# grahamstockton87/RayTracingOneWeekendApplication

Hardware: AMD Instinct MI355X
Metric: Msamples/sec (pixels x spp) on RTIOW final scene 1920x1080 (higher is better)
Workload: dtype f64; 1 GPU; book1_final 1920x1080x100spp depth 50 (BASELINE configs[1]); tiles=8x8 px per wave, interleaved over ranks, parallelism=1 GPU, scene_seed=1592598565, render_seed=1, program_ops=1334, reduced=False, variant=0, order=fast (rtk_scene_upload_fast; proven bit-identical), frames_in_flight=1

## Files before the change

raytracingoneweekendapplication_amd/csrc/rtk_optimize.cpp:

```cpp
#include <algorithm>
#include <cmath>
#include <cstdlib>
#include <cstring>
#include <limits>
#include <new>
#include <unordered_set>
#include <utility>
#include <vector>

#include "rtk.h"

namespace {

struct Box {
    double lo[3], hi[3];
    static Box empty() {
        const double inf = std::numeric_limits<double>::infinity();
        return Box{{inf, inf, inf}, {-inf, -inf, -inf}};
    }
    void grow(const Box& o) {
        for (int a = 0; a < 3; a++) {
            lo[a] = std::min(lo[a], o.lo[a]);
            hi[a] = std::max(hi[a], o.hi[a]);
        }
    }
    void grow(double x, double y, double z) {
        const double p[3] = {x, y, z};
        for (int a = 0; a < 3; a++) {
            lo[a] = std::min(lo[a], p[a]);
            hi[a] = std::max(hi[a], p[a]);
        }
    }
    bool valid() const { return lo[0] <= hi[0] && lo[1] <= hi[1] && lo[2] <= hi[2]; }
    double area() const {
        if (!valid()) return 0.0;
        const double dx = hi[0] - lo[0], dy = hi[1] - lo[1], dz = hi[2] - lo[2];
        return 2.0 * (dx * dy + dy * dz + dz * dx);
    }
    double centre(int a) const { return 0.5 * (lo[a] + hi[a]); }
    double distance2(const double p[3]) const {
        double d2 = 0;
        for (int a = 0; a < 3; a++) {
            const double d = p[a] < lo[a] ? lo[a] - p[a] : (p[a] > hi[a] ? p[a] - hi[a] : 0.0);
            d2 += d * d;
        }
        return d2;
    }
};

struct Item {
    int32_t node;
    Box box;
    double cost;
};

struct Holder {
    rtk_scene_desc desc;
    std::vector<rtk_node> nodes;
    std::vector<int32_t> children;
    std::vector<rtk_aabb> boxes;
};

struct Optimizer {
    const rtk_scene_desc& in;
    const rtk_optimize_opts& opts;
    Holder& out;
    std::vector<int32_t> memo;
    std::vector<Box> memo_box;
    std::vector<double> memo_cost;
    std::vector<char> on_stack;
    std::vector<char> memo_media;
    std::vector<int32_t> ref_rank;
    std::vector<char> holds_medium;
    bool keep_media_order = true;
    int32_t n_ordered = 0;
    bool failed = false;
    bool has_media = false;
    double margin = 0.0, tri_margin = 0.0;
    int split_depth = 0;
    bool has_triangles = false;
    int64_t n_bvh_in = 0;

    Optimizer(const rtk_scene_desc& i, const rtk_optimize_opts& o, Holder& h)
        : in(i), opts(o), out(h), memo(size_t(i.n_nodes), -1), memo_box(size_t(i.n_nodes)), memo_cost(size_t(i.n_nodes), 1.0), on_stack(size_t(i.n_nodes), 0), memo_media(size_t(i.n_nodes), 0) {}

    static constexpr double kBoxCost = 1.0;
    static constexpr double kChainCost = 3.0;
    double prim_cost(int32_t kind) const { return opts.prim_cost_scale * base_prim_cost(kind); }
    static double base_prim_cost(int32_t kind) {
        switch (kind) {
            case RTK_NODE_SPHERE: return 2.1;
            case RTK_NODE_QUAD: return 1.75;
            case RTK_NODE_TRIANGLE: return 1.75;
            default: return 4.0;
        }
    }

    int32_t fail_node() {
        failed = true;
        return -1;
    }
    int32_t push_node(int32_t kind, int32_t a, int32_t b, int32_t c) {
        out.nodes.push_back(rtk_node{kind, a, b, c});
        return int32_t(out.nodes.size()) - 1;
    }

    static void pad_axis(double& lo, double& hi) {
        const double delta = 0.0001;
        if (hi - lo < delta) {
            const double padding = delta / 2;
            lo -= padding;
            hi += padding;
        }
    }
    bool primitive_box(const rtk_node& n, Box& b) {
        b = Box::empty();
        if (n.kind == RTK_NODE_SPHERE) {
            if (n.a < 0 || n.a >= in.n_spheres) return false;
            const rtk_sphere& s = in.spheres[n.a];
            const double r = s.radius;
            b.grow(s.center0.x - r, s.center0.y - r, s.center0.z - r);
            b.grow(s.center0.x + r, s.center0.y + r, s.center0.z + r);
            const double ex = s.center0.x + s.center_dir.x, ey = s.center0.y + s.center_dir.y, ez = s.center0.z + s.center_dir.z;
            b.grow(ex - r, ey - r, ez - r);
            b.grow(ex + r, ey + r, ez + r);
        } else if (n.kind == RTK_NODE_QUAD) {
            if (n.a < 0 || n.a >= in.n_quads) return false;
            const rtk_quad& q = in.quads[n.a];
            b.grow(q.Q.x, q.Q.y, q.Q.z);
            b.grow(q.Q.x + q.u.x, q.Q.y + q.u.y, q.Q.z + q.u.z);
            b.grow(q.Q.x + q.v.x, q.Q.y + q.v.y, q.Q.z + q.v.z);
            b.grow(q.Q.x + q.u.x + q.v.x, q.Q.y + q.u.y + q.v.y, q.Q.z + q.u.z + q.v.z);
        } else {
            if (n.a < 0 || n.a >= in.n_triangles) return false;
            const rtk_triangle& t = in.triangles[n.a];
            b.grow(t.p0.x, t.p0.y, t.p0.z);
            b.grow(t.p1.x, t.p1.y, t.p1.z);
            b.grow(t.p2.x, t.p2.y, t.p2.z);
        }
        for (int a = 0; a < 3; a++) pad_axis(b.lo[a], b.hi[a]);
        if (n.kind == RTK_NODE_TRIANGLE) {
            b = grown(b, tri_margin);
        }
        return true;
    }

    bool gather(int32_t node, std::vector<Item>& items, std::unordered_set<int32_t>& present, int depth) {
        if (failed || node < 0 || node >= in.n_nodes || depth > 4096) return !(failed = true);
        const rtk_node& n = in.nodes[node];
        if (n.kind == RTK_NODE_LIST) {
            if (n.a < 0 || n.b < 0 || int64_t(n.a) + n.b > in.n_list_children) return !(failed = true);
            for (int32_t k = 0; k < n.b; k++)
                if (!gather(in.list_children[n.a + k], items, present, depth + 1)) return false;
            return true;
        }
        if (n.kind == RTK_NODE_BVH) {
            n_bvh_in++;
            return gather(n.a, items, present, depth + 1) && gather(n.b, items, present, depth + 1);
        }
        Box b;
        double cost;
        const int32_t o = convert(node, b, cost, depth + 1);
        if (o < 0) return false;
        if (!present.insert(o).second && !memo_media[node]) return true;
        items.push_back(Item{o, b, cost});
        return true;
    }

    int32_t convert(int32_t node, Box& box, double& cost, int depth) {
        if (failed || node < 0 || node >= in.n_nodes || depth > 4096) {
            failed = true;
            return -1;
        }
        if (memo[node] >= 0) {
            box = memo_box[node];
            cost = memo_cost[node];
            if (memo_media[node]) has_media = true;
            return memo[node];
        }
        if (on_stack[node]) {
            failed = true;
            return -1;
        }
        on_stack[node] = 1;
        const rtk_node& n = in.nodes[node];
        int32_t o = -1;
        switch (n.kind) {
            case RTK_NODE_SPHERE:
            case RTK_NODE_QUAD:
            case RTK_NODE_TRIANGLE:
                if (n.kind == RTK_NODE_TRIANGLE) has_triangles = true;
                if (!primitive_box(n, box)) {
                    failed = true;
                    break;
                }
                cost = prim_cost(n.kind);
                o = push_node(n.kind, n.a, n.b, ref_rank[size_t(node)]);
                break;
            case RTK_NODE_LIST:
            case RTK_NODE_BVH: {
                if (keep_media_order && holds_medium[size_t(node)]) {
                    o = ordered_group(node, box, cost, depth);
                    memo_media[node] = 1;
                    has_media = true;
                    break;
                }
                const bool media_before = has_media;
                has_media = false;
                o = build_group(node, box, cost, depth);
                memo_media[node] = has_media ? 1 : 0;
                has_media = has_media || media_before;
                break;
            }
            case RTK_NODE_TRANSLATE: {
                if (n.a < 0 || n.a >= in.n_translates) {
                    failed = true;
                    break;
                }
                Box cb;
                double cc;
                const int32_t child = convert(n.b, cb, cc, depth + 1);
                if (child < 0) break;
                const rtk_vec3& off = in.translates[n.a].offset;
                box = cb;
                box.lo[0] += off.x; box.hi[0] += off.x;
                box.lo[1] += off.y; box.hi[1] += off.y;
                box.lo[2] += off.z; box.hi[2] += off.z;
                cost = cc + kChainCost;
                o = push_node(RTK_NODE_TRANSLATE, n.a, child, 0);
                memo_media[node] = memo_media[n.b];
                break;
            }
            case RTK_NODE_ROTATE_Y: {
                if (n.a < 0 || n.a >= in.n_rotates) {
                    failed = true;
                    break;
                }
                Box cb;
                double cc;
                const int32_t child = convert(n.b, cb, cc, depth + 1);
                if (child < 0) break;
                const double s = in.rotates[n.a].sin_theta, c = in.rotates[n.a].cos_theta;
                box = Box::empty();
                for (int i = 0; i < 2; i++)
                    for (int j = 0; j < 2; j++)
                        for (int k = 0; k < 2; k++) {
                            const double x = i ? cb.hi[0] : cb.lo[0], y = j ? cb.hi[1] : cb.lo[1], z = k ? cb.hi[2] : cb.lo[2];
                            box.grow(c * x + s * z, y, -s * x + c * z);
                        }
                cost = cc + kChainCost;
                o = push_node(RTK_NODE_ROTATE_Y, n.a, child, 0);
                memo_media[node] = memo_media[n.b];
                break;
            }
            case RTK_NODE_MEDIUM: {
                if (n.a < 0 || n.a >= in.n_media) {
                    failed = true;
                    break;
                }
                has_media = true;
                Box cb;
                double cc;
                const int32_t child = convert(n.b, cb, cc, depth + 1);
                if (child < 0) break;
                box = cb;
                cost = 2.0 * cc + 3.0;
                o = push_node(RTK_NODE_MEDIUM, n.a, child, 0);
                memo_media[node] = 1;
                break;
            }
            default: failed = true; break;
        }
        on_stack[node] = 0;
        if (o < 0) {
            failed = true;
            return -1;
        }
        for (int a = 0; a < 3; a++) {
            const bool empty_axis = !(box.lo[a] <= box.hi[a]);
            const bool nan_axis = box.lo[a] != box.lo[a] || box.hi[a] != box.hi[a];
            if (nan_axis || (!empty_axis && (std::fabs(box.lo[a]) > 1e150 || std::fabs(box.hi[a]) > 1e150)) || !(cost == cost) || cost > 1e300) {
                failed = true;
                return -1;
            }
        }
        memo[node] = o;
        memo_box[node] = box;
        memo_cost[node] = cost;
        return o;
    }

    static Box grown(const Box& b, double m) {
        Box r = b;
        for (int a = 0; a < 3; a++) {
            r.lo[a] -= m;
            r.hi[a] += m;
        }
        return r;
    }

    int32_t emit_list(const std::vector<Item>& items, size_t begin, size_t end) {
        const int32_t first = int32_t(out.children.size());
        for (size_t k = begin; k < end; k++) out.children.push_back(items[k].node);
        return push_node(RTK_NODE_LIST, first, int32_t(end - begin), 0);
    }

    struct Built {
        int32_t node;
        double cost;
        double first;
    };
    bool flatten = [] {
        const char* e = std::getenv("RTK_OPT_FLATTEN");
        return !(e && e[0] == '0');
    }();

    Built represent(std::vector<Item>& items, size_t begin, size_t end, const Box& parent) {
        if (end - begin == 1) {
            const Item& it = items[begin];
            const double pa = parent.area();
            const double boxed = kBoxCost + (pa > 0 ? std::min(1.0, it.box.area() / pa) : 1.0) * it.cost;
            if (boxed < it.cost) {
                const Box padded = grown(it.box, margin);
                out.boxes.push_back(rtk_aabb{padded.lo[0], padded.hi[0], padded.lo[1], padded.hi[1], padded.lo[2], padded.hi[2]});
                const int32_t nothing = push_node(RTK_NODE_LIST, int32_t(out.children.size()), 0, 0);
                return Built{push_node(RTK_NODE_BVH, it.node, nothing, int32_t(out.boxes.size()) - 1), boxed, kBoxCost};
            }
            return Built{it.node, it.cost, it.cost};
        }
        double linear = 0;
        Box b = Box::empty();
        for (size_t k = begin; k < end; k++) {
            linear += items[k].cost;
            b.grow(items[k].box);
        }
        const size_t nodes_mark = out.nodes.size(), child_mark = out.children.size(), box_mark = out.boxes.size();
        Built l{-1, 0, 0}, r{-1, 0, 0};
        Built inner = split(items, begin, end, b, &l, &r);
        const double pa = parent.area();
        const double pb = pa > 0 ? std::min(1.0, b.area() / pa) : 1.0;
        const double boxed = kBoxCost + pb * inner.cost;
        const double bare = flatten ? pb * inner.cost + (1.0 - pb) * (l.first + r.first) : std::numeric_limits<double>::infinity();
        if (int(end - begin) <= opts.max_leaf && linear <= boxed && linear <= bare) {
            out.nodes.resize(nodes_mark);
            out.children.resize(child_mark);
            out.boxes.resize(box_mark);
            order_items(items, begin, end);
            return Built{emit_list(items, begin, end), linear, linear};
        }
        if (bare < boxed && inner.node == int32_t(out.nodes.size()) - 1 && out.nodes.back().kind == RTK_NODE_BVH &&
            out.nodes.back().c == int32_t(out.boxes.size()) - 1) {
            const int32_t first_member = out.nodes.back().a, second_member = out.nodes.back().b;
            out.nodes.pop_back();
            out.boxes.pop_back();
            const int32_t at = int32_t(out.children.size());
            out.children.push_back(first_member);
            out.children.push_back(second_member);
            return Built{push_node(RTK_NODE_LIST, at, 2, 0), bare, l.first + r.first};
        }
        return Built{inner.node, boxed, kBoxCost};
    }

    void order_items(std::vector<Item>& items, size_t begin, size_t end) {
        if (!opts.has_eye) return;
        const double eye[3] = {opts.eye.x, opts.eye.y, opts.eye.z};
        std::stable_sort(items.begin() + long(begin), items.begin() + long(end),
                         [&](const Item& a, const Item& b) { return key(a.box, eye) < key(b.box, eye); });
    }
    static double key(const Box& b, const double eye[3]) {
        const double c[3] = {b.centre(0) - eye[0], b.centre(1) - eye[1], b.centre(2) - eye[2]};
        return b.distance2(eye) + 1e-6 * (c[0] * c[0] + c[1] * c[1] + c[2] * c[2]);
    }

    Built split(std::vector<Item>& items, size_t begin, size_t end, const Box& b, Built* left_out = nullptr, Built* right_out = nullptr) {
        const size_t n = end - begin;
        int best_axis = -1;
        size_t best_k = 0;
        double best = std::numeric_limits<double>::infinity();
        std::vector<double> right_area(n), right_cost(n);
        for (int axis = 0; axis < 3; axis++) {
            std::sort(items.begin() + long(begin), items.begin() + long(end), [&](const Item& x, const Item& y) {
                const double cx = x.box.centre(axis), cy = y.box.centre(axis);
                return cx != cy ? cx < cy : x.node < y.node;
            });
            Box acc = Box::empty();
            double cost = 0;
            for (size_t k = n; k-- > 1;) {
                acc.grow(items[begin + k].box);
                cost += items[begin + k].cost;
                right_area[k] = acc.area();
                right_cost[k] = cost;
            }
            acc = Box::empty();
            cost = 0;
            for (size_t k = 1; k < n; k++) {
                acc.grow(items[begin + k - 1].box);
                cost += items[begin + k - 1].cost;
                const double c = acc.area() * cost + right_area[k] * right_cost[k];
                if (c < best) {
                    best = c;
                    best_axis = axis;
                    best_k = k;
                }
            }
        }
        if (split_depth > 48 && (best_k == 1 || best_k + 1 == n)) best_k = n / 2;
        if (best_axis < 0) {
            best_axis = 2;
            best_k = n / 2;
        }
        if (best_axis != 2)
            std::sort(items.begin() + long(begin), items.begin() + long(end), [&](const Item& x, const Item& y) {
                const double cx = x.box.centre(best_axis), cy = y.box.centre(best_axis);
                return cx != cy ? cx < cy : x.node < y.node;
            });
        const size_t mid = begin + best_k;
        split_depth++;
        Built l = represent(items, begin, mid, b);
        Built r = represent(items, mid, end, b);
        split_depth--;
        bool swap = false;
        Box lb = Box::empty(), rb = Box::empty();
        for (size_t k = begin; k < mid; k++) lb.grow(items[k].box);
        for (size_t k = mid; k < end; k++) rb.grow(items[k].box);
        if (opts.has_eye) {
            const double eye[3] = {opts.eye.x, opts.eye.y, opts.eye.z};
            swap = key(rb, eye) < key(lb, eye);
        } else {
            swap = rb.area() > lb.area();
        }
        if (swap) std::swap(l, r);
        const Box padded = grown(b, margin);
        out.boxes.push_back(rtk_aabb{padded.lo[0], padded.hi[0], padded.lo[1], padded.hi[1], padded.lo[2], padded.hi[2]});
        const int32_t node = push_node(RTK_NODE_BVH, l.node, r.node, int32_t(out.boxes.size()) - 1);
        if (left_out) *left_out = l;
        if (right_out) *right_out = r;
        return Built{node, l.cost + r.cost, l.first + r.first};
    }

    int32_t build_group(int32_t node, Box& box, double& cost, int depth) {
        std::vector<Item> items;
        std::unordered_set<int32_t> present;
        if (!gather(node, items, present, depth)) return -1;
        return build_items(items, box, cost);
    }

    struct Sequence {
        struct Entry {
            int32_t node;
            Box box;
            double cost;
            bool ordered;
        };
        std::vector<Entry> entries;
        std::vector<Item> run;
        std::unordered_set<int32_t> present;
    };
    bool close_run(Sequence& q) {
        if (q.run.empty()) return true;
        Box rb;
        double rc = 0;
        const int32_t g = build_items(q.run, rb, rc);
        if (g < 0) return false;
        q.entries.push_back({g, rb, rc, false});
        q.run.clear();
        q.present.clear();
        return true;
    }
    bool walk_ordered(int32_t node, Sequence& q, int depth) {
        if (failed || node < 0 || node >= in.n_nodes || depth > 4096) return !(failed = true);
        if (!holds_medium[size_t(node)]) return gather(node, q.run, q.present, depth);
        const rtk_node n = in.nodes[node];
        if (n.kind == RTK_NODE_LIST) {
            if (n.a < 0 || n.b < 0 || int64_t(n.a) + n.b > in.n_list_children) return !(failed = true);
            for (int32_t k = 0; k < n.b; k++)
                if (!walk_ordered(in.list_children[n.a + k], q, depth + 1)) return false;
            return true;
        }
        if (n.kind == RTK_NODE_BVH) {
            n_bvh_in++;
            return walk_ordered(n.a, q, depth + 1) && walk_ordered(n.b, q, depth + 1);
        }
        if (!close_run(q)) return false;
        Box b;
        double c = 0;
        const int32_t o = convert(node, b, c, depth + 1);
        if (o < 0) return false;
        q.entries.push_back({o, b, c, true});
        n_ordered++;
        return true;
    }
    int32_t ordered_group(int32_t node, Box& box, double& cost, int depth) {
        Sequence q;
        if (!walk_ordered(node, q, depth) || !close_run(q)) return -1;
        box = Box::empty();
        for (const auto& e : q.entries) box.grow(e.box);
        cost = 0;
        std::vector<int32_t> members;
        for (const auto& e : q.entries) {
            int32_t member = e.node;
            double c = e.cost;
            const double pa = box.area();
            const double boxed = kBoxCost + (pa > 0 ? std::min(1.0, e.box.area() / pa) : 1.0) * e.cost;
            if (e.ordered && e.box.valid() && boxed < e.cost) {
                const Box padded = grown(e.box, margin);
                out.boxes.push_back(rtk_aabb{padded.lo[0], padded.hi[0], padded.lo[1], padded.hi[1], padded.lo[2], padded.hi[2]});
                const int32_t nothing = push_node(RTK_NODE_LIST, int32_t(out.children.size()), 0, 0);
                member = push_node(RTK_NODE_BVH, e.node, nothing, int32_t(out.boxes.size()) - 1);
                c = boxed;
            }
            members.push_back(member);
            cost += c;
        }
        const int32_t first = int32_t(out.children.size());
        out.children.insert(out.children.end(), members.begin(), members.end());
        return push_node(RTK_NODE_LIST, first, int32_t(members.size()), 0);
    }

    bool scan_media(int32_t root) {
        holds_medium.assign(size_t(in.n_nodes), 0);
        std::vector<char> state(size_t(in.n_nodes), 0);
        std::vector<std::pair<int32_t, int32_t>> stack{{root, 0}};
        auto child_of = [&](const rtk_node& n, int32_t k) -> int32_t {
            switch (n.kind) {
                case RTK_NODE_LIST:
                    if (n.a < 0 || n.b < 0 || int64_t(n.a) + n.b > in.n_list_children) return -2;
                    return k < n.b ? in.list_children[n.a + k] : -1;
                case RTK_NODE_BVH: return k == 0 ? n.a : (k == 1 ? n.b : -1);
                case RTK_NODE_TRANSLATE: case RTK_NODE_ROTATE_Y: case RTK_NODE_MEDIUM: return k == 0 ? n.b : -1;
                default: return -1;
            }
        };
        while (!stack.empty()) {
            auto& [node, next] = stack.back();
            if (node < 0 || node >= in.n_nodes || stack.size() > 4100) return false;
            const rtk_node& n = in.nodes[node];
            if (next == 0) {
                if (state[size_t(node)] == 2) { stack.pop_back(); continue; }
                if (state[size_t(node)] == 1) return false;
                state[size_t(node)] = 1;
                if (n.kind == RTK_NODE_MEDIUM) holds_medium[size_t(node)] = 1;
            }
            const int32_t c = child_of(n, next);
            if (c == -2) return false;
            if (c == -1) {
                state[size_t(node)] = 2;
                const int32_t done = node;
                stack.pop_back();
                if (!stack.empty() && holds_medium[size_t(done)]) holds_medium[size_t(stack.back().first)] = 1;
                continue;
            }
            next++;
            if (c < 0 || c >= in.n_nodes) return false;
            if (state[size_t(c)] == 2) {
                if (holds_medium[size_t(c)]) holds_medium[size_t(node)] = 1;
                continue;
            }
            stack.push_back({c, 0});
        }
        return true;
    }

    int32_t build_items(std::vector<Item>& items, Box& box, double& cost) {
        if (items.empty()) {
            box = Box::empty();
            cost = 0;
            return push_node(RTK_NODE_LIST, int32_t(out.children.size()), 0, 0);
        }
        box = Box::empty();
        double linear = 0;
        for (const Item& it : items) {
            box.grow(it.box);
            linear += it.cost;
        }
        if (items.size() == 1) {
            cost = items[0].cost;
            return items[0].node;
        }
        const size_t nodes_mark = out.nodes.size(), child_mark = out.children.size(), box_mark = out.boxes.size();
        Built inner = split(items, 0, items.size(), box);
        if (int(items.size()) <= opts.max_leaf && linear <= kBoxCost + inner.cost) {
            out.nodes.resize(nodes_mark);
            out.children.resize(child_mark);
            out.boxes.resize(box_mark);
            order_items(items, 0, items.size());
            cost = linear;
            return emit_list(items, 0, items.size());
        }
        cost = kBoxCost + inner.cost;
        return inner.node;
    }

    void compute_ranks(int32_t root) {
        ref_rank.assign(size_t(in.n_nodes), 0);
        std::vector<char> seen(size_t(in.n_nodes), 0);
        std::vector<int32_t> stack{root};
        int32_t next = 1;
        size_t guard = 0;
        while (!stack.empty() && guard++ < (size_t(1) << 26)) {
            const int32_t node = stack.back();
            stack.pop_back();
            if (node < 0 || node >= in.n_nodes || seen[size_t(node)]) continue;
            seen[size_t(node)] = 1;
            const rtk_node& n = in.nodes[node];
            switch (n.kind) {
                case RTK_NODE_SPHERE: case RTK_NODE_QUAD: case RTK_NODE_TRIANGLE: ref_rank[size_t(node)] = next++; break;
                case RTK_NODE_LIST:
                    if (n.a >= 0 && n.b >= 0 && int64_t(n.a) + n.b <= in.n_list_children)
                        for (int32_t k = n.b; k-- > 0;) stack.push_back(in.list_children[n.a + k]);
                    break;
                case RTK_NODE_BVH: stack.push_back(n.b); stack.push_back(n.a); break;
                case RTK_NODE_TRANSLATE: case RTK_NODE_ROTATE_Y: case RTK_NODE_MEDIUM: stack.push_back(n.b); break;
                default: break;
            }
        }
    }

    void compute_margin() {
        double extent = 0;
        for (int32_t i = 0; i < in.n_nodes; i++) {
            const rtk_node& n = in.nodes[i];
            if (n.kind == RTK_NODE_SPHERE || n.kind == RTK_NODE_QUAD || n.kind == RTK_NODE_TRIANGLE) {
                Box b;
                if (!primitive_box(n, b)) continue;
                for (int a = 0; a < 3; a++) extent = std::max(extent, std::max(std::fabs(b.lo[a]), std::fabs(b.hi[a])));
            }
        }
        for (int32_t i = 0; i < in.n_translates; i++)
            extent += std::fabs(in.translates[i].offset.x) + std::fabs(in.translates[i].offset.y) + std::fabs(in.translates[i].offset.z);
        if (opts.has_eye) extent = std::max(extent, std::max(std::fabs(opts.eye.x), std::max(std::fabs(opts.eye.y), std::fabs(opts.eye.z))));
        margin = std::ldexp(extent > 0 ? extent : 1.0, -40);
        tri_margin = std::ldexp(extent > 0 ? extent : 1.0, -20);
    }
};

}

namespace rtk {
size_t hot_program_lds_bytes(const rtk_scene_desc* scene);
}

extern "C" {

static int optimize_once(const rtk_scene_desc* scene, const rtk_optimize_opts* opts_in, rtk_scene_desc** out_scene, rtk_optimize_info* info) {
    if (!scene || !out_scene) return RTK_ERR_INVALID;
    *out_scene = nullptr;
    if (scene->abi_version != RTK_ABI_VERSION || scene->n_nodes <= 0 || !scene->nodes || scene->root < 0 || scene->root >= scene->n_nodes) return RTK_ERR_INVALID;
    rtk_optimize_opts opts;
    std::memset(&opts, 0, sizeof opts);
    if (opts_in) opts = *opts_in;
    if (opts.max_leaf <= 0) opts.max_leaf = 4;
    if (!(opts.prim_cost_scale > 0)) opts.prim_cost_scale = 1.0;
    Holder* h = new (std::nothrow) Holder;
    if (!h) return RTK_ERR_INVALID;
    Optimizer op(*scene, opts, *h);
    op.keep_media_order = opts.free_media_order == 0;
    if (!op.scan_media(scene->root)) {
        delete h;
        return RTK_ERR_INVALID;
    }
    op.compute_ranks(scene->root);
    op.compute_margin();
    Box box;
    double cost = 0;
    int32_t root = op.convert(scene->root, box, cost, 0);
    if (root < 0 || op.failed) {
        delete h;
        return RTK_ERR_INVALID;
    }
    if (h->nodes[size_t(root)].kind != RTK_NODE_LIST && h->nodes[size_t(root)].kind != RTK_NODE_BVH) {
        const int32_t first = int32_t(h->children.size());
        h->children.push_back(root);
        root = op.push_node(RTK_NODE_LIST, first, 1, 0);
    }
    if (h->nodes[size_t(root)].kind == RTK_NODE_BVH && opts.has_eye) {
        const rtk_node rn = h->nodes[size_t(root)];
        const rtk_aabb& rb = h->boxes[size_t(rn.c)];
        const bool inside = opts.eye.x > rb.xmin && opts.eye.x < rb.xmax && opts.eye.y > rb.ymin && opts.eye.y < rb.ymax && opts.eye.z > rb.zmin &&
                            opts.eye.z < rb.zmax;
        const double lo[3] = {rb.xmin, rb.ymin, rb.zmin}, hi[3] = {rb.xmax, rb.ymax, rb.zmax}, e[3] = {opts.eye.x, opts.eye.y, opts.eye.z};
        double dist2 = 0, diag2 = 0;
        for (int a = 0; a < 3; a++) {
            const double d = e[a] < lo[a] ? lo[a] - e[a] : (e[a] > hi[a] ? e[a] - hi[a] : 0.0);
            dist2 += d * d;
            diag2 += (hi[a] - lo[a]) * (hi[a] - lo[a]);
        }
        const bool near_by = op.flatten && dist2 < diag2;
        if (inside || near_by) {
            const int32_t first = int32_t(h->children.size());
            h->children.push_back(rn.a);
            h->children.push_back(rn.b);
            root = op.push_node(RTK_NODE_LIST, first, 2, 0);
        }
    }
    h->desc = *scene;
    h->desc.root = root;
    h->desc.n_nodes = int32_t(h->nodes.size());
    h->desc.nodes = h->nodes.data();
    h->desc.n_list_children = int32_t(h->children.size());
    h->desc.list_children = h->children.data();
    h->desc.n_bvh_boxes = int32_t(h->boxes.size());
    h->desc.bvh_boxes = h->boxes.data();
    if (info) {
        info->exact = (op.has_media && !op.keep_media_order) ? 0 : (op.has_triangles ? 1 : 2);
        info->has_media = op.has_media ? 1 : 0;
        info->n_ordered_items = op.n_ordered;
        info->has_triangles = op.has_triangles ? 1 : 0;
        info->n_bvh_nodes_in = int32_t(op.n_bvh_in);
        info->n_bvh_nodes_out = int32_t(h->boxes.size());
        info->expected_cost = cost;
        info->box_margin = op.margin;
    }
    *out_scene = &h->desc;
    return RTK_OK;
}

void rtk_scene_optimized_free(rtk_scene_desc* scene) { delete reinterpret_cast<Holder*>(scene); }

static size_t compact_program_bytes(const rtk_scene_desc& d, bool mixed_layout = false) {
    size_t bytes = 32  + size_t(d.n_materials) * 48;
    std::vector<std::pair<int32_t, int>> stack{{d.root, 0}};
    size_t guard = 0;
    while (!stack.empty() && guard++ < (size_t(1) << 24) && bytes < (size_t(1) << 30)) {
        const auto [node, depth] = stack.back();
        stack.pop_back();
        if (node < 0 || node >= d.n_nodes || depth > 4096) continue;
        const rtk_node& n = d.nodes[node];
        switch (n.kind) {
            case RTK_NODE_SPHERE: {
                const bool moving = n.a >= 0 && n.a < d.n_spheres && (d.spheres[n.a].center_dir.x != 0 || d.spheres[n.a].center_dir.y != 0 || d.spheres[n.a].center_dir.z != 0);
                bytes += mixed_layout ? (moving ? 96 : 64) : (moving ? 80 : 48);
                break;
            }
            case RTK_NODE_QUAD: bytes += 144; break;
            case RTK_NODE_TRIANGLE: bytes += 80; break;
            case RTK_NODE_LIST:
                if (n.a >= 0 && n.b >= 0 && int64_t(n.a) + n.b <= d.n_list_children)
                    for (int32_t k = 0; k < n.b; k++) stack.push_back({d.list_children[n.a + k], depth + 1});
                break;
            case RTK_NODE_BVH: bytes += 32; stack.push_back({n.a, depth + 1}); stack.push_back({n.b, depth + 1}); break;
            case RTK_NODE_TRANSLATE: case RTK_NODE_ROTATE_Y: bytes += 64; stack.push_back({n.b, depth + 1}); break;
            case RTK_NODE_MEDIUM: {
                const bool sphere_bound = n.b >= 0 && n.b < d.n_nodes && d.nodes[n.b].kind == RTK_NODE_SPHERE;
                if (sphere_bound) bytes += 48;
                else { bytes += 96; stack.push_back({n.b, depth + 1}); stack.push_back({n.b, depth + 1}); }
                break;
            }
            default: break;
        }
    }
    return bytes;
}

static void slot_program_counts(const rtk_scene_desc& d, size_t& n_slots, size_t& n_boxes) {
    n_slots = 1;
    n_boxes = 0;
    std::vector<std::pair<int32_t, int>> stack{{d.root, 0}};
    size_t guard = 0;
    while (!stack.empty() && guard++ < (size_t(1) << 24) && n_slots < (size_t(1) << 26)) {
        const auto [node, depth] = stack.back();
        stack.pop_back();
        if (node < 0 || node >= d.n_nodes || depth > 4096) continue;
        const rtk_node& n = d.nodes[node];
        switch (n.kind) {
            case RTK_NODE_SPHERE: {
                const bool moving = n.a >= 0 && n.a < d.n_spheres && (d.spheres[n.a].center_dir.x != 0 || d.spheres[n.a].center_dir.y != 0 || d.spheres[n.a].center_dir.z != 0);
                n_slots += moving ? 2 : 1;
                break;
            }
            case RTK_NODE_QUAD: n_slots += 3; break;
            case RTK_NODE_TRIANGLE: n_slots += 2; break;
            case RTK_NODE_LIST:
                if (n.a >= 0 && n.b >= 0 && int64_t(n.a) + n.b <= d.n_list_children)
                    for (int32_t k = 0; k < n.b; k++) stack.push_back({d.list_children[n.a + k], depth + 1});
                break;
            case RTK_NODE_BVH: n_slots++; n_boxes++; stack.push_back({n.a, depth + 1}); stack.push_back({n.b, depth + 1}); break;
            case RTK_NODE_TRANSLATE: case RTK_NODE_ROTATE_Y: n_slots += 2; stack.push_back({n.b, depth + 1}); break;
            case RTK_NODE_MEDIUM: {
                const bool sphere_bound = n.b >= 0 && n.b < d.n_nodes && d.nodes[n.b].kind == RTK_NODE_SPHERE;
                if (sphere_bound) n_slots++;
                else { n_slots += 3; stack.push_back({n.b, depth + 1}); stack.push_back({n.b, depth + 1}); }
                break;
            }
            default: break;
        }
    }
}

static bool gets_mixed_program(const rtk_scene_desc& d) {
    if (d.n_quads > 0 || d.n_triangles > 0 || d.n_media > 0 || d.n_translates > 0 || d.n_rotates > 0 || d.n_lights > 0) return false;
    for (int32_t i = 0; i < d.n_materials; i++) {
        const rtk_material& m = d.materials[i];
        if (m.kind != RTK_MAT_LAMBERTIAN && m.kind != RTK_MAT_METAL && m.kind != RTK_MAT_DIELECTRIC) return false;
        if (m.kind == RTK_MAT_LAMBERTIAN && (m.texture < 0 || m.texture >= d.n_textures || d.textures[m.texture].kind != RTK_TEX_SOLID)) return false;
    }
    return true;
}

int rtk_scene_optimize(const rtk_scene_desc* scene, const rtk_optimize_opts* opts_in, rtk_scene_desc** out_scene, rtk_optimize_info* info) {
    if (!scene || !out_scene) return RTK_ERR_INVALID;
    rtk_optimize_opts o;
    std::memset(&o, 0, sizeof o);
    if (opts_in) o = *opts_in;
    if (o.prim_cost_scale > 0) return optimize_once(scene, &o, out_scene, info);
    const size_t budget = size_t(160) * 1024 - 2048;
    static const double kScalesNoQuads[] = {1.5, 1.4, 1.2, 1.0, 0.85, 0.7, 0.6, 0.5, 0.4};
    static const double kScalesQuads[] = {2.0, 1.0, 0.85, 0.7, 0.6, 0.5, 0.4};
    const double* kScales = scene->n_quads == 0 ? kScalesNoQuads : kScalesQuads;
    const int n_scales = scene->n_quads == 0 ? int(sizeof kScalesNoQuads / sizeof kScalesNoQuads[0]) : int(sizeof kScalesQuads / sizeof kScalesQuads[0]);
    const bool full_feature = scene->n_media > 0 || scene->n_translates > 0 || scene->n_rotates > 0;
    const bool mixed_layout = gets_mixed_program(*scene);
    rtk_scene_desc* fallback = nullptr;
    rtk_optimize_info fallback_info;
    for (int k = 0; k < n_scales; k++) {
        o.prim_cost_scale = kScales[k];
        rtk_optimize_info local;
        rtk_scene_desc* candidate = nullptr;
        const int rc = optimize_once(scene, &o, &candidate, &local);
        if (rc != RTK_OK) {
            if (fallback) rtk_scene_optimized_free(fallback);
            return rc;
        }
        bool accept = compact_program_bytes(*candidate, mixed_layout) <= budget;
        if (!accept && kScales[k] <= 1.0 && full_feature) {
            const size_t hot = rtk::hot_program_lds_bytes(candidate);
            accept = hot > 0 && hot + size_t(scene->n_perlins) * 9216 <= budget;
        }
        if (accept) {
            if (fallback) rtk_scene_optimized_free(fallback);
            *out_scene = candidate;
            if (info) *info = local;
            return RTK_OK;
        }
        bool keep = false;
        if (!fallback && kScales[k] <= 1.0) {
            size_t n_slots = 0, n_boxes = 0;
            slot_program_counts(*candidate, n_slots, n_boxes);
            const size_t whole = n_slots * 64 + size_t(scene->n_materials) * 48;
            const size_t boxes_only = n_boxes * 56 + n_slots / 2 + n_slots / 4 + 64 + 2048;
            keep = whole <= budget || boxes_only <= budget || k + 1 == n_scales;
        }
        if (keep || (!fallback && k + 1 == n_scales)) {
            fallback = candidate;
            fallback_info = local;
        } else {
            rtk_scene_optimized_free(candidate);
        }
        if (fallback && !full_feature) break;
    }
    if (!fallback) return RTK_ERR_INVALID;
    *out_scene = fallback;
    if (info) *info = fallback_info;
    return RTK_OK;
}

}
```

Measured before the change: 11520 Msamples/s.

## Price BVH node entry with sampled pilot rays instead of surface area

Adds a pilot ray set built from sample primitive surfaces (cosine-weighted directions from their normals) plus camera rays to the eye. The BVH builder estimates the chance of entering a child box as the fraction of parent rays that hit it, falling back to the surface-area ratio when rays are few or the estimate is unreliable. The aim is a tree whose box and flatten decisions match the actual ray distribution, cutting traversal cost per sample. It adds build-time cost, and the heuristic could produce a worse tree for real path-traced rays.

```diff
diff --git a/raytracingoneweekendapplication_amd/csrc/rtk_optimize.cpp b/raytracingoneweekendapplication_amd/csrc/rtk_optimize.cpp
--- a/raytracingoneweekendapplication_amd/csrc/rtk_optimize.cpp
+++ b/raytracingoneweekendapplication_amd/csrc/rtk_optimize.cpp
@@ -219,7 +219,9 @@
                 }
                 Box cb;
                 double cc;
+                xform_depth++;
                 const int32_t child = convert(n.b, cb, cc, depth + 1);
+                xform_depth--;
                 if (child < 0) break;
                 const rtk_vec3& off = in.translates[n.a].offset;
                 box = cb;
@@ -238,7 +240,9 @@
                 }
                 Box cb;
                 double cc;
+                xform_depth++;
                 const int32_t child = convert(n.b, cb, cc, depth + 1);
+                xform_depth--;
                 if (child < 0) break;
                 const double s = in.rotates[n.a].sin_theta, c = in.rotates[n.a].cos_theta;
                 box = Box::empty();
@@ -315,11 +319,161 @@
         return !(e && e[0] == '0');
     }();
 
-    Built represent(std::vector<Item>& items, size_t begin, size_t end, const Box& parent) {
+    struct PilotRay {
+        double o[3], d[3], w;
+    };
+    std::vector<PilotRay> pilot;
+    int xform_depth = 0;
+    static constexpr int kPilotDirs = 16;
+    static constexpr size_t kPilotPrimitives = 256;
+    static constexpr double kLooseShare = 0.001;
+    static constexpr size_t kPilotMinRays = 64;
+    bool surface_pricing = [] {
+        const char* e = std::getenv("RTK_OPT_SURFACE");
+        return !(e && e[0] == '0');
+    }();
+
+    void add_pilot_origin(const double p[3], const double n_in[3]) {
+        const double len = std::sqrt(n_in[0] * n_in[0] + n_in[1] * n_in[1] + n_in[2] * n_in[2]);
+        if (!(len > 0) || !(len < 1e300)) return;
+        const double n[3] = {n_in[0] / len, n_in[1] / len, n_in[2] / len};
+        const int h = std::fabs(n[0]) <= std::fabs(n[1]) && std::fabs(n[0]) <= std::fabs(n[2]) ? 0 : (std::fabs(n[1]) <= std::fabs(n[2]) ? 1 : 2);
+        double e[3] = {0, 0, 0};
+        e[h] = 1.0;
+        double t[3] = {n[1] * e[2] - n[2] * e[1], n[2] * e[0] - n[0] * e[2], n[0] * e[1] - n[1] * e[0]};
+        const double tl = std::sqrt(t[0] * t[0] + t[1] * t[1] + t[2] * t[2]);
+        for (int a = 0; a < 3; a++) t[a] /= tl;
+        const double b[3] = {n[1] * t[2] - n[2] * t[1], n[2] * t[0] - n[0] * t[2], n[0] * t[1] - n[1] * t[0]};
+        for (int k = 0; k < kPilotDirs; k++) {
+            const double u = (k + 0.5) / kPilotDirs, cos_t = std::sqrt(1.0 - u), sin_t = std::sqrt(u);
+            const double phi = 6.283185307179586 * std::fmod(k * 0.6180339887498949, 1.0);
+            const double x = sin_t * std::cos(phi), y = sin_t * std::sin(phi);
+            PilotRay r;
+            for (int a = 0; a < 3; a++) {
+                r.o[a] = p[a];
+                r.d[a] = x * t[a] + y * b[a] + cos_t * n[a];
+            }
+            r.w = 1.0;
+            pilot.push_back(r);
+        }
+        if (opts.has_eye) {
+            const double eye[3] = {opts.eye.x, opts.eye.y, opts.eye.z};
+            const double d[3] = {p[0] - eye[0], p[1] - eye[1], p[2] - eye[2]};
+            const double dl = std::sqrt(d[0] * d[0] + d[1] * d[1] + d[2] * d[2]);
+            if (dl > 0 && dl < 1e300) pilot.push_back(PilotRay{{eye[0], eye[1], eye[2]}, {d[0] / dl, d[1] / dl, d[2] / dl}, 0.5 * kPilotDirs});
+        }
+    }
+    void build_pilot(int32_t root) {
+        pilot.clear();
+        if (!surface_pricing) return;
+        std::vector<int32_t> prims, stack{root};
+        std::vector<char> seen(size_t(in.n_nodes), 0);
+        size_t guard = 0;
+        while (!stack.empty() && guard++ < (size_t(1) << 26)) {
+            const int32_t node = stack.back();
+            stack.pop_back();
+            if (node < 0 || node >= in.n_nodes || seen[size_t(node)]) continue;
+            seen[size_t(node)] = 1;
+            const rtk_node& n = in.nodes[node];
+            switch (n.kind) {
+                case RTK_NODE_SPHERE: if (n.a >= 0 && n.a < in.n_spheres) prims.push_back(node); break;
+                case RTK_NODE_QUAD: if (n.a >= 0 && n.a < in.n_quads) prims.push_back(node); break;
+                case RTK_NODE_TRIANGLE: if (n.a >= 0 && n.a < in.n_triangles) prims.push_back(node); break;
+                case RTK_NODE_LIST:
+                    if (n.a >= 0 && n.b >= 0 && int64_t(n.a) + n.b <= in.n_list_children)
+                        for (int32_t k = n.b; k-- > 0;) stack.push_back(in.list_children[n.a + k]);
+                    break;
+                case RTK_NODE_BVH: stack.push_back(n.b); stack.push_back(n.a); break;
+                default: break;
+            }
+        }
+        const size_t stride = (prims.size() + kPilotPrimitives - 1) / kPilotPrimitives;
+        for (size_t i = 0; i < prims.size(); i += std::max<size_t>(stride, 1)) {
+            const rtk_node& n = in.nodes[prims[i]];
+            if (n.kind == RTK_NODE_SPHERE) {
+                const rtk_sphere& s = in.spheres[n.a];
+                for (int a = 0; a < 3; a++)
+                    for (int sign = -1; sign <= 1; sign += 2) {
+                        double p[3] = {s.center0.x, s.center0.y, s.center0.z}, nrm[3] = {0, 0, 0};
+                        p[a] += sign * s.radius;
+                        nrm[a] = sign;
+                        add_pilot_origin(p, nrm);
+                    }
+                continue;
+            }
+            double p[3], u[3], v[3];
+            if (n.kind == RTK_NODE_QUAD) {
+                const rtk_quad& q = in.quads[n.a];
+                const double Q[3] = {q.Q.x, q.Q.y, q.Q.z}, qu[3] = {q.u.x, q.u.y, q.u.z}, qv[3] = {q.v.x, q.v.y, q.v.z};
+                for (int a = 0; a < 3; a++) {
+                    u[a] = qu[a];
+                    v[a] = qv[a];
+                    p[a] = Q[a] + 0.5 * (qu[a] + qv[a]);
+                }
+            } else {
+                const rtk_triangle& t = in.triangles[n.a];
+                const double p0[3] = {t.p0.x, t.p0.y, t.p0.z}, p1[3] = {t.p1.x, t.p1.y, t.p1.z}, p2[3] = {t.p2.x, t.p2.y, t.p2.z};
+                for (int a = 0; a < 3; a++) {
+                    u[a] = p1[a] - p0[a];
+                    v[a] = p2[a] - p0[a];
+                    p[a] = (p0[a] + p1[a] + p2[a]) / 3.0;
+                }
+            }
+            const double nrm[3] = {u[1] * v[2] - u[2] * v[1], u[2] * v[0] - u[0] * v[2], u[0] * v[1] - u[1] * v[0]};
+            const double back[3] = {-nrm[0], -nrm[1], -nrm[2]};
+            add_pilot_origin(p, nrm);
+            add_pilot_origin(p, back);
+        }
+    }
+    static bool enters(const PilotRay& r, const Box& b, double t_min = 0.001) {
+        double t0 = t_min, t1 = std::numeric_limits<double>::infinity();
+        for (int a = 0; a < 3; a++) {
+            if (r.d[a] == 0) {
+                if (r.o[a] < b.lo[a] || r.o[a] > b.hi[a]) return false;
+                continue;
+            }
+            const double inv = 1.0 / r.d[a];
+            double ta = (b.lo[a] - r.o[a]) * inv, tb = (b.hi[a] - r.o[a]) * inv;
+            if (ta > tb) std::swap(ta, tb);
+            t0 = std::max(t0, ta);
+            t1 = std::min(t1, tb);
+            if (t1 <= t0) return false;
+        }
+        return true;
+    }
+    using Rays = std::vector<uint32_t>;
+    Rays rays_entering(const Rays& from, const Box& b) const {
+        const Box padded = grown(b, margin);
+        Rays kept;
+        for (uint32_t k : from)
+            if (enters(pilot[k], padded)) kept.push_back(k);
+        return kept;
+    }
+    double weight(const Rays& rays) const {
+        double w = 0;
+        for (uint32_t k : rays) w += pilot[k].w;
+        return w;
+    }
+    double enter_chance(const Box& inner, const Box& parent, const Rays* in_parent, const Rays* in_inner = nullptr) const {
+        const double pa = parent.area();
+        const double by_area = pa > 0 ? std::min(1.0, inner.area() / pa) : 1.0;
+        if (!in_parent || in_parent->size() < kPilotMinRays || !inner.valid()) return by_area;
+        const double met = in_inner ? weight(*in_inner) : weight(rays_entering(*in_parent, inner)), all = weight(*in_parent);
+        if (!(all > 0)) return by_area;
+        if (!in_inner) {
+            double loose = 0;
+            const Box wide = grown(inner, std::ldexp(margin, 21));
+            for (uint32_t k : *in_parent)
+                if (enters(pilot[k], wide, 0.0)) loose += pilot[k].w;
+            if (loose - met > kLooseShare * all) return by_area;
+        }
+        return std::min(by_area, met / all);
+    }
+
+    Built represent(std::vector<Item>& items, size_t begin, size_t end, const Box& parent, const Rays* in_parent) {
         if (end - begin == 1) {
             const Item& it = items[begin];
-            const double pa = parent.area();
-            const double boxed = kBoxCost + (pa > 0 ? std::min(1.0, it.box.area() / pa) : 1.0) * it.cost;
+            const double boxed = kBoxCost + enter_chance(it.box, parent, in_parent) * it.cost;
             if (boxed < it.cost) {
                 const Box padded = grown(it.box, margin);
                 out.boxes.push_back(rtk_aabb{padded.lo[0], padded.hi[0], padded.lo[1], padded.hi[1], padded.lo[2], padded.hi[2]});
@@ -336,9 +490,10 @@
         }
         const size_t nodes_mark = out.nodes.size(), child_mark = out.children.size(), box_mark = out.boxes.size();
         Built l{-1, 0, 0}, r{-1, 0, 0};
-        Built inner = split(items, begin, end, b, &l, &r);
-        const double pa = parent.area();
-        const double pb = pa > 0 ? std::min(1.0, b.area() / pa) : 1.0;
+        Rays mine;
+        if (in_parent) mine = rays_entering(*in_parent, b);
+        Built inner = split(items, begin, end, b, in_parent ? &mine : nullptr, &l, &r);
+        const double pb = enter_chance(b, parent, in_parent, &mine);
         const double boxed = kBoxCost + pb * inner.cost;
         const double bare = flatten ? pb * inner.cost + (1.0 - pb) * (l.first + r.first) : std::numeric_limits<double>::infinity();
         if (int(end - begin) <= opts.max_leaf && linear <= boxed && linear <= bare) {
@@ -372,7 +527,7 @@
         return b.distance2(eye) + 1e-6 * (c[0] * c[0] + c[1] * c[1] + c[2] * c[2]);
     }
 
-    Built split(std::vector<Item>& items, size_t begin, size_t end, const Box& b, Built* left_out = nullptr, Built* right_out = nullptr) {
+    Built split(std::vector<Item>& items, size_t begin, size_t end, const Box& b, const Rays* inside, Built* left_out = nullptr, Built* right_out = nullptr) {
         const size_t n = end - begin;
         int best_axis = -1;
         size_t best_k = 0;
@@ -416,8 +571,9 @@
             });
         const size_t mid = begin + best_k;
         split_depth++;
-        Built l = represent(items, begin, mid, b);
-        Built r = represent(items, mid, end, b);
+        if (split_depth > 48) inside = nullptr;
+        Built l = represent(items, begin, mid, b, inside);
+        Built r = represent(items, mid, end, b, inside);
         split_depth--;
         bool swap = false;
         Box lb = Box::empty(), rb = Box::empty();
@@ -578,7 +734,14 @@
             return items[0].node;
         }
         const size_t nodes_mark = out.nodes.size(), child_mark = out.children.size(), box_mark = out.boxes.size();
-        Built inner = split(items, 0, items.size(), box);
+        Rays inside;
+        const bool piloted = !pilot.empty() && xform_depth == 0;
+        if (piloted) {
+            Rays every(pilot.size());
+            for (size_t k = 0; k < every.size(); k++) every[k] = uint32_t(k);
+            inside = rays_entering(every, box);
+        }
+        Built inner = split(items, 0, items.size(), box, piloted ? &inside : nullptr);
         if (int(items.size()) <= opts.max_leaf && linear <= kBoxCost + inner.cost) {
             out.nodes.resize(nodes_mark);
             out.children.resize(child_mark);
@@ -661,6 +824,7 @@
     }
     op.compute_ranks(scene->root);
     op.compute_margin();
+    op.build_pilot(scene->root);
     Box box;
     double cost = 0;
     int32_t root = op.convert(scene->root, box, cost, 0);
```

Measured after the change: 11620 Msamples/s, median of 6. Within noise of the previous version (+0.9%).
